# frank-xwang/InstanceDiffusion

Hardware: AMD Instinct MI355X
Metric: images/sec at 512x512, 50 PLMS steps, N=8 instances (Multi-instance Sampler) (higher is better)
Workload: dtype bf16; 1 GPU; C3: SD-1.5 InstanceDiffusion UNet (1.228B params, seeded random weights), 64x64 latent (512x512), 50 PLMS steps, CFG 7.5, N=8 boxes, MIS 0.36, alpha [0.8,0,0.2]; images_per_gpu=32, unet_forwards_per_image=406

## Files before the change

### instancediffusion_amd/csrc/proj320_stream.hip

```cpp
#include "mw_row.h"

using namespace idfcore;
using namespace idfmw;

namespace {

constexpr int PS_BM = 32, PS_C = 320;
constexpr int PS_MIN_ROWS_PER_CU = 512;
constexpr int PS_P = 3;
constexpr int PS_NX = 3, PS_NR = 4;
constexpr int PS_SLOT = 5 * 32 * 128;
constexpr int PS_RO_OFF = PS_NX * PS_SLOT, PS_ST_OFF = PS_RO_OFF + PS_NR * PS_SLOT;
constexpr int PS_SMEM = PS_ST_OFF + PS_NX * 256;
enum { PS_PLAIN = 0, PS_RES = 1, PS_LN = 2 };

struct PsParams {
  const unsigned short* x; int ldx;
  const unsigned short* w; int ldw;
  const float* bias;
  const float* c; const float* ln_stats;
  const unsigned short* res; int ldr;
  const float* gate;
  unsigned short* out; int ldo;
  float* out_stats; float eps;
  int M;
};

__device__ __forceinline__ void ps_dma16(const void* sbase , unsigned voff, unsigned lds ) {
  lds = __builtin_amdgcn_readfirstlane(lds);
  asm volatile("s_mov_b32 m0, %0\n\ts_nop 0\n\tglobal_load_lds_dwordx4 %1, %2" ::"s"(lds), "v"(voff), "s"(sbase) : "memory", "m0");
}
__device__ __forceinline__ void ps_dma4(const void* sbase , unsigned voff, unsigned lds ) {
  lds = __builtin_amdgcn_readfirstlane(lds);
  asm volatile("s_mov_b32 m0, %0\n\ts_nop 0\n\tglobal_load_lds_dword %1, %2" ::"s"(lds), "v"(voff), "s"(sbase) : "memory", "m0");
}
template <int F, int OFF> __device__ __forceinline__ void ps_load_w(const unsigned short* rowp) {
  asm volatile("global_load_dwordx4 a[%c1:%c2], %0, off offset:%c3" ::"v"(rowp), "n"(4 * F), "n"(4 * F + 3), "n"(OFF) : "memory");
}
template <int DT, int F, bool FIRST> __device__ __forceinline__ void ps_mfma(f32x4& acc, const u32x4& x) {
  if constexpr (FIRST) {
    if constexpr (DT == IDF_BF16) asm volatile("v_mfma_f32_16x16x32_bf16 %0, a[%c2:%c3], %1, 0" : "=&v"(acc) : "v"(x), "n"(4 * F), "n"(4 * F + 3));
    else asm volatile("v_mfma_f32_16x16x32_f16 %0, a[%c2:%c3], %1, 0" : "=&v"(acc) : "v"(x), "n"(4 * F), "n"(4 * F + 3));
  } else {
    if constexpr (DT == IDF_BF16) asm volatile("v_mfma_f32_16x16x32_bf16 %0, a[%c2:%c3], %1, %0" : "+v"(acc) : "v"(x), "n"(4 * F), "n"(4 * F + 3));
    else asm volatile("v_mfma_f32_16x16x32_f16 %0, a[%c2:%c3], %1, %0" : "+v"(acc) : "v"(x), "n"(4 * F), "n"(4 * F + 3));
  }
}
template <int OFF> __device__ __forceinline__ void ps_store16(unsigned voff, const u32x4& v, const void* sbase ) {
  asm volatile("global_store_dwordx4 %0, %1, %2 offset:%c3" ::"v"(voff), "v"(v), "s"(sbase), "n"(OFF) : "memory");
}
__device__ __forceinline__ void ps_store8(unsigned voff, const f32x2& v, const void* sbase ) {
  asm volatile("global_store_dwordx2 %0, %1, %2" ::"v"(voff), "v"(v), "s"(sbase) : "memory");
}

template <int DT, int MODE, bool STATS>
__global__ __launch_bounds__(256, 1) void proj320s_kernel(const PsParams p, const int blocks) {
  asm volatile("" ::: "a0", "a199");
  extern __shared__ __attribute__((aligned(128))) char smem[];
  constexpr bool RES = MODE == PS_RES, LN = MODE == PS_LN;
  constexpr int NLOAD = 5 + (RES ? 5 : 0) + (LN ? 1 : 0), NSTORE = 5 + (STATS ? 1 : 0);
  constexpr int VMC = PS_P * NSTORE + (PS_P - 1) * NLOAD;
  static_assert(VMC < 64, "vmcnt is a 6-bit counter");
  const RowLane rl = mw_row_lane();
  const int tid = rl.tid, lane = rl.lane, wave = rl.wave, l15 = lane & 15, q = lane >> 4;
  const int G = gridDim.x;
  const unsigned smem_lds = lds_u32(smem);

  const int blk0 = mw_first_tile(G);
  if (blk0 >= blocks) return;
  const int nblk = (blocks - blk0 + G - 1) / G;

  f32x4 bias[5], cc[5];
#pragma unroll
  for (int nt = 0; nt < 5; ++nt) {
    bias[nt] = *reinterpret_cast<const f32x4*>(p.bias + 80 * wave + 16 * nt + 4 * q);
    if constexpr (LN) cc[nt] = *reinterpret_cast<const f32x4*>(p.c + 80 * wave + 16 * nt + 4 * q);
  }
  float gm = 1.0f;
  if constexpr (RES) if (p.gate) gm = p.gate[0];
#pragma unroll
  for (int nt = 0; nt < 5; ++nt) {
    asm volatile("" : "+v"(bias[nt]));
    if constexpr (LN) asm volatile("" : "+v"(cc[nt]));
  }
  asm volatile("" : "+v"(gm));

  const int prow = 8 * wave + (lane >> 3);
  const unsigned pswz = (unsigned)((((lane & 7) ^ ((prow >> 1) & 7)) << 4));
  const unsigned x_voff = (unsigned)(prow * p.ldx * 2) + pswz;
  const unsigned r_voff = RES ? (unsigned)(prow * p.ldr * 2) + pswz : 0u;
  auto issue = [&](int i) {
    const int ii = i < nblk ? i : nblk - 1;
    const size_t m0 = (size_t)(blk0 + ii * G) * PS_BM;
    const char* xb = reinterpret_cast<const char*>(p.x) + m0 * p.ldx * 2;
    const unsigned xs = smem_lds + (unsigned)((i % PS_NX) * PS_SLOT + wave * 1024);
#pragma unroll
    for (int kt = 0; kt < 5; ++kt) ps_dma16(xb + kt * 128, x_voff, xs + (unsigned)(kt * 4096));
    if constexpr (RES) {
      const char* rb = reinterpret_cast<const char*>(p.res) + m0 * p.ldr * 2;
      const unsigned rs = smem_lds + (unsigned)(PS_RO_OFF + (i % PS_NR) * PS_SLOT + wave * 1024);
#pragma unroll
      for (int kt = 0; kt < 5; ++kt) ps_dma16(rb + kt * 128, r_voff, rs + (unsigned)(kt * 4096));
    }
    if constexpr (LN)
      ps_dma4(reinterpret_cast<const char*>(p.ln_stats + 2 * m0), (unsigned)(lane * 4), smem_lds + (unsigned)(PS_ST_OFF + (i % PS_NX) * 256));
  };

#pragma unroll
  for (int i = 0; i < PS_P; ++i) issue(i);
  {
    const unsigned short* wp = p.w + (size_t)(80 * wave + l15) * p.ldw + 8 * q;
    mw_static_for<5>([&](auto nt) {
      const unsigned short* wr = wp + (size_t)(16 * decltype(nt)::value) * p.ldw;
      mw_static_for<10>([&](auto ks) { ps_load_w<decltype(nt)::value * 10 + decltype(ks)::value, 64 * decltype(ks)::value>(wr); });
    });
  }
  asm volatile("s_waitcnt vmcnt(0)" ::: "memory");

  unsigned xoff[2][2], eoff[2][5];
#pragma unroll
  for (int mt = 0; mt < 2; ++mt) {
    const int row = 16 * mt + l15, sw = (row >> 1) & 7;
#pragma unroll
    for (int h = 0; h < 2; ++h) xoff[mt][h] = (unsigned)(row * 128 + (((4 * h + q) ^ sw) << 4));
#pragma unroll
    for (int nt = 0; nt < 5; ++nt) {
      const int n = 80 * wave + 16 * nt + 4 * q;
      eoff[mt][nt] = (unsigned)((n >> 6) * 4096 + row * 128 + ((((n & 63) >> 3) ^ sw) << 4) + (n & 7) * 2);
    }
  }
  const int crow = tid >> 3, cj = tid & 7;
  const unsigned coff = (unsigned)(crow * 128 + ((cj ^ ((crow >> 1) & 7)) << 4));
  const unsigned o_voff = (unsigned)(crow * p.ldo * 2 + cj * 16);

  for (int i = 0; i < nblk; ++i) {
    asm volatile("s_waitcnt vmcnt(%c0)\n\ts_barrier" ::"n"(VMC) : "memory");
    const char* xs = smem + (i % PS_NX) * PS_SLOT;
    char* ro = smem + PS_RO_OFF + (i % PS_NR) * PS_SLOT;
    const size_t m0 = (size_t)(blk0 + i * G) * PS_BM;

    u32x4 xf[2][10];
#pragma unroll
    for (int ks = 0; ks < 10; ++ks)
#pragma unroll
      for (int mt = 0; mt < 2; ++mt) xf[mt][ks] = *reinterpret_cast<const u32x4*>(xs + xoff[mt][ks & 1] + (ks >> 1) * 4096);
    f32x4 acc[2][5];
    mw_static_for<10>([&](auto ks) {
      mw_static_for<5>([&](auto nt) {
        constexpr int KS = decltype(ks)::value, NT = decltype(nt)::value;
        ps_mfma<DT, NT * 10 + KS, KS == 0>(acc[0][NT], xf[0][KS]);
        ps_mfma<DT, NT * 10 + KS, KS == 0>(acc[1][NT], xf[1][KS]);
      });
    });
    asm volatile("s_nop 15\n\ts_nop 15"
                 : "+v"(acc[0][0]), "+v"(acc[0][1]), "+v"(acc[0][2]), "+v"(acc[0][3]), "+v"(acc[0][4]), "+v"(acc[1][0]), "+v"(acc[1][1]),
                   "+v"(acc[1][2]), "+v"(acc[1][3]), "+v"(acc[1][4]));

#pragma unroll
    for (int mt = 0; mt < 2; ++mt) {
      f32x2 st = {0.0f, 1.0f};
      if constexpr (LN) st = *reinterpret_cast<const f32x2*>(smem + PS_ST_OFF + (i % PS_NX) * 256 + (16 * mt + l15) * 8);
#pragma unroll
      for (int nt = 0; nt < 5; ++nt) {
        float v[4];
#pragma unroll
        for (int r = 0; r < 4; ++r) {
          v[r] = acc[mt][nt][r];
          if constexpr (LN) v[r] = st[1] * fmaf(-st[0], cc[nt][r], v[r]);
          v[r] += bias[nt][r];
        }
        if constexpr (RES) {
          const u32x2 rr = *reinterpret_cast<const u32x2*>(ro + eoff[mt][nt]);
#pragma unroll
          for (int h = 0; h < 2; ++h) {
            v[2 * h] = fmaf(gm, v[2 * h], Elem<DT>::to_f32((unsigned short)(rr[h] & 0xffffu)));
            v[2 * h + 1] = fmaf(gm, v[2 * h + 1], Elem<DT>::to_f32((unsigned short)(rr[h] >> 16)));
          }
        }
        *reinterpret_cast<u32x2*>(ro + eoff[mt][nt]) = u32x2{pack2<DT>(v[0], v[1]), pack2<DT>(v[2], v[3])};
      }
    }
    asm volatile("s_waitcnt lgkmcnt(0)\n\ts_barrier" ::: "memory");

    issue(i + PS_P);

    u32x4 o[5];
#pragma unroll
    for (int kt = 0; kt < 5; ++kt) o[kt] = *reinterpret_cast<const u32x4*>(ro + coff + kt * 4096);
    const char* ob = reinterpret_cast<const char*>(p.out) + m0 * p.ldo * 2;
    ps_store16<0>(o_voff, o[0], ob);
    ps_store16<128>(o_voff, o[1], ob);
    ps_store16<256>(o_voff, o[2], ob);
    ps_store16<384>(o_voff, o[3], ob);
    ps_store16<512>(o_voff, o[4], ob);
    if constexpr (STATS) {
      float f[40];
#pragma unroll
      for (int kt = 0; kt < 5; ++kt) unpack8<DT>(o[kt], f + 8 * kt);
      float sum = 0.0f;
#pragma unroll
      for (int e = 0; e < 40; ++e) sum += f[e];
      sum += __shfl_xor(sum, 1, 64); sum += __shfl_xor(sum, 2, 64); sum += __shfl_xor(sum, 4, 64);
      const float mean = sum * (1.0f / PS_C);
      float m2 = 0.0f;
#pragma unroll
      for (int e = 0; e < 40; ++e) { const float d = f[e] - mean; m2 = fmaf(d, d, m2); }
      m2 += __shfl_xor(m2, 1, 64); m2 += __shfl_xor(m2, 2, 64); m2 += __shfl_xor(m2, 4, 64);
      const f32x2 mr = {mean, rsqrtf(m2 * (1.0f / PS_C) + p.eps)};
      if (cj == 0) ps_store8((unsigned)(crow * 8), mr, reinterpret_cast<const char*>(p.out_stats + 2 * m0));
    }
  }
  asm volatile("s_waitcnt vmcnt(0)" ::: "memory");
}

template <int DT>
int ps_launch(const PsParams& q, int mode, hipStream_t s) {
  const bool st = q.out_stats != nullptr;
  if (mode == PS_PLAIN) return st ? mw_row_launch<PsParams, proj320s_kernel<DT, PS_PLAIN, true>, PS_SMEM, PS_BM>(q, s)
                                  : mw_row_launch<PsParams, proj320s_kernel<DT, PS_PLAIN, false>, PS_SMEM, PS_BM>(q, s);
  if (mode == PS_RES) return st ? mw_row_launch<PsParams, proj320s_kernel<DT, PS_RES, true>, PS_SMEM, PS_BM>(q, s)
                                : mw_row_launch<PsParams, proj320s_kernel<DT, PS_RES, false>, PS_SMEM, PS_BM>(q, s);
  return st ? mw_row_launch<PsParams, proj320s_kernel<DT, PS_LN, true>, PS_SMEM, PS_BM>(q, s)
            : mw_row_launch<PsParams, proj320s_kernel<DT, PS_LN, false>, PS_SMEM, PS_BM>(q, s);
}

}

MwKnob idf_proj_row_knob{"IDF_PROJ_ROW", 1};
int idf_projw_set_mode(int v) { return idf_proj_row_knob.set(v); }
int idf_projw_min_rows() {
  static int per_cu = 0;
  if (per_cu == 0) {
    const char* e = getenv("IDF_PROJ_MIN_ROWS_PER_CU");
    const int v = e ? atoi(e) : PS_MIN_ROWS_PER_CU;
    per_cu = (v < 2 * PS_BM || v % (2 * PS_BM)) ? PS_MIN_ROWS_PER_CU : v;
  }
  return idf_proj_row_knob.get() ? per_cu * idf_num_cu() : 0;
}

int idf_launch_proj320s(const idfcore::CoreParams& p, int dtype, float* out_stats, float out_stats_eps, hipStream_t s) {
  if (idf_proj_row_knob.get() == 0) return IDF_BIG_UNSUPPORTED;
  if (p.K != PS_C || p.N != PS_C || !p.out || p.vt_out) return IDF_BIG_UNSUPPORTED;
  if ((p.M % PS_BM) || p.M < idf_projw_min_rows()) return IDF_BIG_UNSUPPORTED;
  if (dtype != IDF_BF16 && dtype != IDF_F16) return IDF_BIG_UNSUPPORTED;
  int mode;
  if (p.epi == IDF_EPI_BIAS) mode = PS_PLAIN;
  else if (p.epi == (IDF_EPI_BIAS | IDF_EPI_RES) || p.epi == (IDF_EPI_BIAS | IDF_EPI_RES | IDF_EPI_GATE)) mode = PS_RES;
  else if (p.epi == (IDF_EPI_BIAS | IDF_EPI_LN_ROW)) mode = PS_LN;
  else return IDF_BIG_UNSUPPORTED;
  if (!p.bias || !aligned16(p.bias)) return IDF_BIG_UNSUPPORTED;
  if (mode == PS_LN && (!p.ln_stats || p.stride_ln_stats || !p.ln_c || !aligned16(p.ln_c) || (((uintptr_t)p.ln_stats) & 7u))) return IDF_BIG_UNSUPPORTED;
  if (mode == PS_RES && (!p.res || !aligned16(p.res) || p.ldr < PS_C || (p.ldr % 8))) return IDF_BIG_UNSUPPORTED;
  if ((p.epi & IDF_EPI_GATE) && !p.gate) return IDF_BIG_UNSUPPORTED;
  if (p.lda < PS_C || p.ldw < PS_C || p.ldo < PS_C || (p.lda % 8) || (p.ldw % 8) || (p.ldo % 8)) return IDF_BIG_UNSUPPORTED;
  if (!aligned16(p.A) || !aligned16(p.W) || !aligned16(p.out)) return IDF_BIG_UNSUPPORTED;
  if (out_stats && (((uintptr_t)out_stats) & 7u)) return IDF_BIG_UNSUPPORTED;
  const long long ldmax = p.lda > p.ldo ? (p.lda > p.ldr ? p.lda : p.ldr) : (p.ldo > p.ldr ? p.ldo : p.ldr);
  if ((long long)PS_C * p.ldw * 2 >= (1ll << 31) || (long long)PS_BM * ldmax * 2 >= (1ll << 31)) return IDF_BIG_UNSUPPORTED;
  if (p.out == (const void*)p.A && p.ldo != p.lda) return IDF_BIG_UNSUPPORTED;
  if (mode == PS_RES && p.out == (const void*)p.res && p.ldo != p.ldr) return IDF_BIG_UNSUPPORTED;
  PsParams q;
  q.x = p.A; q.ldx = p.lda; q.w = p.W; q.ldw = p.ldw; q.bias = p.bias; q.c = p.ln_c; q.ln_stats = p.ln_stats;
  q.res = p.res; q.ldr = p.ldr; q.gate = (p.epi & IDF_EPI_GATE) ? p.gate : nullptr;
  q.out = static_cast<unsigned short*>(p.out); q.ldo = p.ldo; q.out_stats = out_stats; q.eps = out_stats_eps; q.M = p.M;
  return dtype == IDF_BF16 ? ps_launch<IDF_BF16>(q, mode, s) : ps_launch<IDF_F16>(q, mode, s);
}
```

Measured before the change: 2.146 img/s.

## Interleave previous block's epilogue stores and next prefetch into MFMA loop

Restructures the streaming proj320 kernel so that the LDS reads, global stores and LayerNorm-stats computation of the previous block, plus the DMA prefetch of the next block, are spread across the 50 MFMA slots of the current block through sched_barrier hook points. Residual and LN-stat LDS reads are also hoisted into the MFMA loop, and the lane reductions switch from shuffles to DPP. This removes the separate epilogue barrier and store phase, aiming to hide memory and LDS latency behind matrix work. Prefetch depth drops from 3 to 2 with an adjusted vmcnt. It also adds PS_DROP debug macros and s_nop after stores, and the tighter vmcnt and ring-slot reuse carry a correctness risk.

```diff
diff --git a/instancediffusion_amd/csrc/proj320_stream.hip b/instancediffusion_amd/csrc/proj320_stream.hip
--- a/instancediffusion_amd/csrc/proj320_stream.hip
+++ b/instancediffusion_amd/csrc/proj320_stream.hip
@@ -7,7 +7,7 @@
 
 constexpr int PS_BM = 32, PS_C = 320;
 constexpr int PS_MIN_ROWS_PER_CU = 512;
-constexpr int PS_P = 3;
+constexpr int PS_P = 2;
 constexpr int PS_NX = 3, PS_NR = 4;
 constexpr int PS_SLOT = 5 * 32 * 128;
 constexpr int PS_RO_OFF = PS_NX * PS_SLOT, PS_ST_OFF = PS_RO_OFF + PS_NR * PS_SLOT;
@@ -47,11 +47,25 @@
   }
 }
 template <int OFF> __device__ __forceinline__ void ps_store16(unsigned voff, const u32x4& v, const void* sbase ) {
-  asm volatile("global_store_dwordx4 %0, %1, %2 offset:%c3" ::"v"(voff), "v"(v), "s"(sbase), "n"(OFF) : "memory");
+  asm volatile("global_store_dwordx4 %0, %1, %2 offset:%c3\n\ts_nop 1" ::"v"(voff), "v"(v), "s"(sbase), "n"(OFF) : "memory");
+}
+__device__ __forceinline__ float ps_row8_sum(float v) {
+  auto dpp = [](float x, auto ctrl) {
+    const int i = __builtin_bit_cast(int, x);
+    return __builtin_bit_cast(float, __builtin_amdgcn_update_dpp(i, i, decltype(ctrl)::value, 0xf, 0xf, false));
+  };
+  v += dpp(v, std::integral_constant<int, 0xB1>{});
+  v += dpp(v, std::integral_constant<int, 0x4E>{});
+  v += dpp(v, std::integral_constant<int, 0x141>{});
+  return v;
 }
 __device__ __forceinline__ void ps_store8(unsigned voff, const f32x2& v, const void* sbase ) {
   asm volatile("global_store_dwordx2 %0, %1, %2" ::"v"(voff), "v"(v), "s"(sbase) : "memory");
 }
+
+#ifndef PS_DROP
+#define PS_DROP 0
+#endif
 
 template <int DT, int MODE, bool STATS>
 __global__ __launch_bounds__(256, 1) void proj320s_kernel(const PsParams p, const int blocks) {
@@ -59,8 +73,9 @@
   extern __shared__ __attribute__((aligned(128))) char smem[];
   constexpr bool RES = MODE == PS_RES, LN = MODE == PS_LN;
   constexpr int NLOAD = 5 + (RES ? 5 : 0) + (LN ? 1 : 0), NSTORE = 5 + (STATS ? 1 : 0);
-  constexpr int VMC = PS_P * NSTORE + (PS_P - 1) * NLOAD;
+  constexpr int VMC = NSTORE + NLOAD;
   static_assert(VMC < 64, "vmcnt is a 6-bit counter");
+  static_assert(10 + NLOAD <= 21, "the hook points of the block loop");
   const RowLane rl = mw_row_lane();
   const int tid = rl.tid, lane = rl.lane, wave = rl.wave, l15 = lane & 15, q = lane >> 4;
   const int G = gridDim.x;
@@ -89,25 +104,32 @@
   const unsigned pswz = (unsigned)((((lane & 7) ^ ((prow >> 1) & 7)) << 4));
   const unsigned x_voff = (unsigned)(prow * p.ldx * 2) + pswz;
   const unsigned r_voff = RES ? (unsigned)(prow * p.ldr * 2) + pswz : 0u;
-  auto issue = [&](int i) {
+  struct Src { const char* xb; const char* rb; const char* sb; unsigned xs, rs, ss; };
+  auto source = [&](int i) {
     const int ii = i < nblk ? i : nblk - 1;
     const size_t m0 = (size_t)(blk0 + ii * G) * PS_BM;
-    const char* xb = reinterpret_cast<const char*>(p.x) + m0 * p.ldx * 2;
-    const unsigned xs = smem_lds + (unsigned)((i % PS_NX) * PS_SLOT + wave * 1024);
-#pragma unroll
-    for (int kt = 0; kt < 5; ++kt) ps_dma16(xb + kt * 128, x_voff, xs + (unsigned)(kt * 4096));
-    if constexpr (RES) {
-      const char* rb = reinterpret_cast<const char*>(p.res) + m0 * p.ldr * 2;
-      const unsigned rs = smem_lds + (unsigned)(PS_RO_OFF + (i % PS_NR) * PS_SLOT + wave * 1024);
-#pragma unroll
-      for (int kt = 0; kt < 5; ++kt) ps_dma16(rb + kt * 128, r_voff, rs + (unsigned)(kt * 4096));
-    }
-    if constexpr (LN)
-      ps_dma4(reinterpret_cast<const char*>(p.ln_stats + 2 * m0), (unsigned)(lane * 4), smem_lds + (unsigned)(PS_ST_OFF + (i % PS_NX) * 256));
+    Src s;
+    s.xb = reinterpret_cast<const char*>(p.x) + m0 * p.ldx * 2;
+    s.xs = smem_lds + (unsigned)((i % PS_NX) * PS_SLOT + wave * 1024);
+    s.rb = RES ? reinterpret_cast<const char*>(p.res) + m0 * p.ldr * 2 : nullptr;
+    s.rs = smem_lds + (unsigned)(PS_RO_OFF + (i % PS_NR) * PS_SLOT + wave * 1024);
+    s.sb = LN ? reinterpret_cast<const char*>(p.ln_stats + 2 * m0) : nullptr;
+    s.ss = smem_lds + (unsigned)(PS_ST_OFF + (i % PS_NX) * 256);
+    return s;
   };
-
-#pragma unroll
-  for (int i = 0; i < PS_P; ++i) issue(i);
+  auto piece = [&](const Src& s, auto jc) {
+    constexpr int J = decltype(jc)::value;
+    if constexpr (J < 5) ps_dma16(s.xb + J * 128, x_voff, s.xs + (unsigned)(J * 4096));
+    else if constexpr (RES) ps_dma16(s.rb + (J - 5) * 128, r_voff, s.rs + (unsigned)((J - 5) * 4096));
+    else
+      ps_dma4(s.sb, (unsigned)(lane * 4), s.ss);
+  };
+
+#pragma unroll
+  for (int i = 0; i < PS_P; ++i) {
+    const Src s = source(i);
+    mw_static_for<NLOAD>([&](auto j) { piece(s, j); });
+  }
   {
     const unsigned short* wp = p.w + (size_t)(80 * wave + l15) * p.ldw + 8 * q;
     mw_static_for<5>([&](auto nt) {
@@ -133,23 +155,69 @@
   const unsigned coff = (unsigned)(crow * 128 + ((cj ^ ((crow >> 1) & 7)) << 4));
   const unsigned o_voff = (unsigned)(crow * p.ldo * 2 + cj * 16);
 
-  for (int i = 0; i < nblk; ++i) {
-    asm volatile("s_waitcnt vmcnt(%c0)\n\ts_barrier" ::"n"(VMC) : "memory");
+  auto block = [&](const int i, auto firstc) {
+    constexpr bool FIRST = decltype(firstc)::value;
+    asm volatile("s_waitcnt vmcnt(%c0) lgkmcnt(0)\n\ts_barrier" ::"n"(VMC) : "memory");
     const char* xs = smem + (i % PS_NX) * PS_SLOT;
     char* ro = smem + PS_RO_OFF + (i % PS_NR) * PS_SLOT;
-    const size_t m0 = (size_t)(blk0 + i * G) * PS_BM;
+    const char* rp = smem + PS_RO_OFF + ((i + PS_NR - 1) % PS_NR) * PS_SLOT;
+    const size_t mp = (size_t)(blk0 + (i - 1) * G) * PS_BM;
+    const char* obp = reinterpret_cast<const char*>(p.out) + mp * p.ldo * 2;
+    const Src nx = source(i + PS_P);
 
     u32x4 xf[2][10];
 #pragma unroll
     for (int ks = 0; ks < 10; ++ks)
 #pragma unroll
       for (int mt = 0; mt < 2; ++mt) xf[mt][ks] = *reinterpret_cast<const u32x4*>(xs + xoff[mt][ks & 1] + (ks >> 1) * 4096);
+    __builtin_amdgcn_sched_barrier(0);
+
+    u32x4 o[5];
+    float f[40], sum = 0.0f, mean = 0.0f, m2 = 0.0f;
+    u32x2 rr[2][5];
+    f32x2 st[2] = {{0.0f, 1.0f}, {0.0f, 1.0f}};
+    auto hook = [&](auto ptc) {
+      constexpr int PT = decltype(ptc)::value;
+      if constexpr (!FIRST && PT < 5) o[PT] = *reinterpret_cast<const u32x4*>(rp + coff + PT * 4096);
+      if constexpr (!FIRST && PT >= 5 && PT < 10 && !(PS_DROP & 1)) ps_store16<128 * (PT - 5)>(o_voff, o[PT - 5], obp);
+      if constexpr (PT >= 10 && PT < 10 + NLOAD && !(PS_DROP & 2)) piece(nx, std::integral_constant<int, PT - 10>{});
+      if constexpr (!FIRST && STATS && !(PS_DROP & 8)) {
+        if constexpr (PT >= 21 && PT < 26) {
+          unpack8<DT>(o[PT - 21], f + 8 * (PT - 21));
+#pragma unroll
+          for (int e = 8 * (PT - 21); e < 8 * (PT - 20); ++e) sum += f[e];
+        }
+        if constexpr (PT == 26) {
+          sum = ps_row8_sum(sum);
+          mean = sum * (1.0f / PS_C);
+        }
+        if constexpr (PT >= 27 && PT < 32) {
+#pragma unroll
+          for (int e = 8 * (PT - 27); e < 8 * (PT - 26); ++e) { const float d = f[e] - mean; m2 = fmaf(d, d, m2); }
+        }
+      }
+      if constexpr (!FIRST && STATS && PT == 32) {
+        m2 = ps_row8_sum(m2);
+        const f32x2 mr = {mean, rsqrtf(m2 * (1.0f / PS_C) + p.eps)};
+        if constexpr (!(PS_DROP & 1))
+          if (cj == 0) ps_store8((unsigned)(crow * 8), mr, reinterpret_cast<const char*>(p.out_stats + 2 * mp));
+      }
+      if constexpr (RES && PT >= 33 && PT < 43) rr[(PT - 33) / 5][(PT - 33) % 5] = *reinterpret_cast<const u32x2*>(ro + eoff[(PT - 33) / 5][(PT - 33) % 5]);
+      if constexpr (LN && PT >= 33 && PT < 35) st[PT - 33] = *reinterpret_cast<const f32x2*>(smem + PS_ST_OFF + (i % PS_NX) * 256 + (16 * (PT - 33) + l15) * 8);
+      if constexpr (PT < 43) __builtin_amdgcn_sched_barrier(0);
+    };
+
     f32x4 acc[2][5];
     mw_static_for<10>([&](auto ks) {
       mw_static_for<5>([&](auto nt) {
         constexpr int KS = decltype(ks)::value, NT = decltype(nt)::value;
-        ps_mfma<DT, NT * 10 + KS, KS == 0>(acc[0][NT], xf[0][KS]);
-        ps_mfma<DT, NT * 10 + KS, KS == 0>(acc[1][NT], xf[1][KS]);
+        if constexpr (PS_DROP & 4) {
+          if constexpr (KS == 0) acc[0][NT] = acc[1][NT] = f32x4{xf[0][NT][0] * 0.0f, 0.0f, 0.0f, 0.0f};
+        } else {
+          ps_mfma<DT, NT * 10 + KS, KS == 0>(acc[0][NT], xf[0][KS]);
+          ps_mfma<DT, NT * 10 + KS, KS == 0>(acc[1][NT], xf[1][KS]);
+        }
+        hook(std::integral_constant<int, KS * 5 + NT>{});
       });
     });
     asm volatile("s_nop 15\n\ts_nop 15"
@@ -158,41 +226,39 @@
 
 #pragma unroll
     for (int mt = 0; mt < 2; ++mt) {
-      f32x2 st = {0.0f, 1.0f};
-      if constexpr (LN) st = *reinterpret_cast<const f32x2*>(smem + PS_ST_OFF + (i % PS_NX) * 256 + (16 * mt + l15) * 8);
 #pragma unroll
       for (int nt = 0; nt < 5; ++nt) {
         float v[4];
 #pragma unroll
         for (int r = 0; r < 4; ++r) {
           v[r] = acc[mt][nt][r];
-          if constexpr (LN) v[r] = st[1] * fmaf(-st[0], cc[nt][r], v[r]);
+          if constexpr (LN) v[r] = st[mt][1] * fmaf(-st[mt][0], cc[nt][r], v[r]);
           v[r] += bias[nt][r];
         }
         if constexpr (RES) {
-          const u32x2 rr = *reinterpret_cast<const u32x2*>(ro + eoff[mt][nt]);
 #pragma unroll
           for (int h = 0; h < 2; ++h) {
-            v[2 * h] = fmaf(gm, v[2 * h], Elem<DT>::to_f32((unsigned short)(rr[h] & 0xffffu)));
-            v[2 * h + 1] = fmaf(gm, v[2 * h + 1], Elem<DT>::to_f32((unsigned short)(rr[h] >> 16)));
+            v[2 * h] = fmaf(gm, v[2 * h], Elem<DT>::to_f32((unsigned short)(rr[mt][nt][h] & 0xffffu)));
+            v[2 * h + 1] = fmaf(gm, v[2 * h + 1], Elem<DT>::to_f32((unsigned short)(rr[mt][nt][h] >> 16)));
           }
         }
         *reinterpret_cast<u32x2*>(ro + eoff[mt][nt]) = u32x2{pack2<DT>(v[0], v[1]), pack2<DT>(v[2], v[3])};
       }
     }
-    asm volatile("s_waitcnt lgkmcnt(0)\n\ts_barrier" ::: "memory");
-
-    issue(i + PS_P);
-
+  };
+
+  block(0, std::true_type{});
+  for (int i = 1; i < nblk; ++i) block(i, std::false_type{});
+
+  asm volatile("s_waitcnt lgkmcnt(0)\n\ts_barrier" ::: "memory");
+  {
+    const char* rp = smem + PS_RO_OFF + ((nblk - 1) % PS_NR) * PS_SLOT;
+    const size_t mp = (size_t)(blk0 + (nblk - 1) * G) * PS_BM;
+    const char* obp = reinterpret_cast<const char*>(p.out) + mp * p.ldo * 2;
     u32x4 o[5];
 #pragma unroll
-    for (int kt = 0; kt < 5; ++kt) o[kt] = *reinterpret_cast<const u32x4*>(ro + coff + kt * 4096);
-    const char* ob = reinterpret_cast<const char*>(p.out) + m0 * p.ldo * 2;
-    ps_store16<0>(o_voff, o[0], ob);
-    ps_store16<128>(o_voff, o[1], ob);
-    ps_store16<256>(o_voff, o[2], ob);
-    ps_store16<384>(o_voff, o[3], ob);
-    ps_store16<512>(o_voff, o[4], ob);
+    for (int kt = 0; kt < 5; ++kt) o[kt] = *reinterpret_cast<const u32x4*>(rp + coff + kt * 4096);
+    if constexpr (!(PS_DROP & 1)) mw_static_for<5>([&](auto kt) { ps_store16<128 * decltype(kt)::value>(o_voff, o[decltype(kt)::value], obp); });
     if constexpr (STATS) {
       float f[40];
 #pragma unroll
@@ -200,14 +266,15 @@
       float sum = 0.0f;
 #pragma unroll
       for (int e = 0; e < 40; ++e) sum += f[e];
-      sum += __shfl_xor(sum, 1, 64); sum += __shfl_xor(sum, 2, 64); sum += __shfl_xor(sum, 4, 64);
+      sum = ps_row8_sum(sum);
       const float mean = sum * (1.0f / PS_C);
       float m2 = 0.0f;
 #pragma unroll
       for (int e = 0; e < 40; ++e) { const float d = f[e] - mean; m2 = fmaf(d, d, m2); }
-      m2 += __shfl_xor(m2, 1, 64); m2 += __shfl_xor(m2, 2, 64); m2 += __shfl_xor(m2, 4, 64);
+      m2 = ps_row8_sum(m2);
       const f32x2 mr = {mean, rsqrtf(m2 * (1.0f / PS_C) + p.eps)};
-      if (cj == 0) ps_store8((unsigned)(crow * 8), mr, reinterpret_cast<const char*>(p.out_stats + 2 * m0));
+      if constexpr (!(PS_DROP & 1))
+        if (cj == 0) ps_store8((unsigned)(crow * 8), mr, reinterpret_cast<const char*>(p.out_stats + 2 * mp));
     }
   }
   asm volatile("s_waitcnt vmcnt(0)" ::: "memory");
```

Result: no change. 2.152 img/s (median of 6 runs) (+0.3%).
